# salesforce/warp-drive

Measured on AMD Instinct MI355X. Metric: env steps/sec, TagContinuous 5 taggers x 100 runners, higher is better.
Workload: dtype f32; 1 GPU; BASELINE configs[2]: TagContinuous 5 taggers x 100 runners, partial obs K=10 (F=71), num_envs=2000 per GPU; tick = sample_actions (2 heads) + step + reset of finished replicas (one fused launch); num_envs_per_gpu=2000, num_agents=105, launch_mode=plan, kernels_per_tick=1, ticks_per_launch=1, parallelism=env-replica sharding x1

## Files before the change

### experiments/phase_profile.py

```python
#!/usr/bin/env python3
import os
import subprocess
import sys

ROOT = os.path.dirname(os.path.dirname(os.path.abspath(__file__)))
sys.path.insert(0, ROOT)
PROF_DIR = os.environ.get("WD_PROF_DIR", os.path.join(ROOT, "build", "variants", "prof"))
if len(sys.argv) > 1 and sys.argv[1] == "build":
    from warp_drive_amd import build as wb

    if os.environ.get("WD_PROF_SRC"):
        wb.KDIR = os.environ["WD_PROF_SRC"]
        wb.KERNEL_FLAGS = [f"-I{wb.KDIR}" if f.startswith("-I") else f for f in wb.KERNEL_FLAGS]

    os.makedirs(PROF_DIR, exist_ok=True)
    for out, (unit, flags) in wb.UNITS.items():
        if out.startswith("wd_kernels_tc_k10"):
            subprocess.run([wb._hipcc(), *wb.KERNEL_FLAGS, *flags, "-DWD_TC_PROBES=1", os.path.join(wb.KDIR, unit), "-o",
                            os.path.join(PROF_DIR, out)], check=True)
            print("built", os.path.join(PROF_DIR, out))
    sys.exit(0)
E = int(sys.argv[1]) if len(sys.argv) > 1 else 2000
T_STAMP = int(sys.argv[2]) if len(sys.argv) > 2 else 300
N_RUNNERS = int(sys.argv[3]) if len(sys.argv) > 3 else 100
N_TICKS = int(sys.argv[4]) if len(sys.argv) > 4 else 32
name = "prof"
os.environ["WD_HSACO_DIR"] = PROF_DIR
os.environ.setdefault("HIP_FORCE_DEV_KERNARG", "1")
import time

import numpy as np
import torch

import bench
from warp_drive_amd.env_wrapper import EnvWrapper
from warp_drive_amd.envs.tag_continuous import TagContinuous
from warp_drive_amd.managers import hip_driver as drv
from warp_drive_amd.managers.function_manager import HIPSampler
from warp_drive_amd.rollout import RolloutEngine
from warp_drive_amd.training.data_loader import create_and_push_data_placeholders

w = EnvWrapper(env_obj=TagContinuous(**dict(bench.BENCH_CFG, num_runners=N_RUNNERS)), num_envs=E, env_backend="hip")
WPB = (w.n_agents + 63) // 64
w.reset_all_envs()
sampler = HIPSampler(w.cuda_function_manager)
sampler.init_random(seed=1)
create_and_push_data_placeholders(env_wrapper=w, action_sampler=sampler, training_batch_size_per_env=None,
                                  push_data_batch_placeholders=False)
engine = RolloutEngine(w, sampler, fused=True)
SLOTS = 24
n_waves = WPB * E
buf = drv.mem_alloc(n_waves * SLOTS * 8)
drv.memset(buf, 0, n_waves * SLOTS * 8)
sym, nbytes = w.cuda_function_manager._module_of(engine.step_kernel_name).get_global("tc_prof_g")
drv.memcpy_htod(sym, np.array([int(buf)], dtype=np.uint64))
engine.run(300)
torch.cuda.synchronize()
t0 = time.perf_counter()
engine.run(1000)
torch.cuda.synchronize()
print(f"=== {name}: wall per tick {(time.perf_counter() - t0) / 1000 * 1e6:.2f} us (stamped build)")
looped = engine.rollout_kernel_name is not None
stamp_trip = N_TICKS // 2 if looped else 0
engine.run((T_STAMP - stamp_trip - 1300) % 500)
torch.cuda.synchronize()
if looped:
    mod = w.cuda_function_manager._module_of(engine.rollout_kernel_name)
    drv.memcpy_htod(mod.get_global("tc_prof_g")[0], np.array([int(buf)], dtype=np.uint64))
    drv.memcpy_htod(mod.get_global("tc_prof_tick_g")[0], np.array([stamp_trip], dtype=np.int32))
    print(f"multi-tick entry {engine.rollout_kernel_name}: a launch of {N_TICKS} ticks, trip {stamp_trip} stamped "
          "(the wavefront counters add up over the whole launch)")
live = w.cuda_data_manager.pull_data_from_device("still_in_the_game").sum(axis=1).mean()
print(f"stamped launch = tick {T_STAMP} of an episode, {live:.1f} agents in the game")
drv.memset(buf, 0, n_waves * SLOTS * 8)
torch.cuda.synchronize()
engine.run(N_TICKS if looped else 1)
torch.cuda.synchronize()
raw = np.zeros(n_waves * SLOTS, dtype=np.uint64)
drv.memcpy_dtoh(raw, buf)
drv.synchronize()
st = raw.reshape(-1, SLOTS).astype(np.int64)
ran = st[:, 15] > 0
searched = st[:, 9] > 0
print(f"wavefronts: {ran.sum()}; ran the search: {searched.sum()}; with a lane in the two-pass fallback / whole-wavefront resolution: "
      f"{(st[:, 20] > 0).sum()}; with a lane whose close pair was settled by one exact compare: "
      f"{(st[:, 23] > 0).sum()}; with a lane in the full ranking: {(st[:, 22] > 0).sum()}")
pre = searched & (st[:, 19] > 0)
if pre.any():
    tr = st[pre, 18]
    print(f"prefiltered wavefronts: {pre.sum()}; radius check failed: {(st[pre, 19] == 2).sum()}; chain trips (pass 2) mean {tr.mean():.1f} "
          f"p50 {np.percentile(tr, 50):.0f} p99 {np.percentile(tr, 99):.0f} max {tr.max()}")
for k in range(1, 16):
    st[:, k] = np.where(st[:, k] > 0, st[:, k], st[:, k - 1])
names = ["start", "loads issued+tables", "sampled", "barrier1", "moved", "barrier2", "tags", "search: radius", "search: prefiltered chain",
         "search: full chain", "search: keys resolved", "search: ids, remember", "id rows + barrier + nearest ids flushed",
         "obs gathered+flushed", "barrier3", "rewards/end"]
if pre.any():
    sp = st[pre]
    print(f"--- all {pre.sum()} prefiltered wavefronts: mean / p10 / p50 / p90 / max shader cycles")
    for k in (7, 8, 9, 10, 11):
        d = sp[:, k] - sp[:, k - 1]
        print(f"  {names[k]:<40} {d.mean():9.0f} {np.percentile(d, 10):9.0f} {np.percentile(d, 50):9.0f} {np.percentile(d, 90):9.0f} {d.max():9.0f}")
    d = sp[:, 11] - sp[:, 6]
    print(f"  {'search, all of it':<40} {d.mean():9.0f} {np.percentile(d, 10):9.0f} {np.percentile(d, 50):9.0f} {np.percentile(d, 90):9.0f} {d.max():9.0f}")
    blk = np.nonzero(pre)[0] // WPB
    slow = np.array([d[blk == b].max() for b in np.unique(blk)])
    print(f"  slowest searcher of each block: mean {slow.mean():.0f} p50 {np.percentile(slow, 50):.0f} p90 {np.percentile(slow, 90):.0f}")
for wv, label in ((0, "wave 0 of each block"), (WPB - 1, "the last wave of each block")):
    s = st[wv::WPB]
    ok = (s[:, 6] > 0) & (s[:, 15] > 0)
    s = s[ok]
    print(f"--- {label}: {ok.sum()} waves; mean / p10 / p90 shader cycles per phase")
    for k in range(1, 16):
        d = s[:, k] - s[:, k - 1]
        print(f"  {names[k]:<40} {d.mean():9.0f} {np.percentile(d, 10):9.0f} {np.percentile(d, 90):9.0f}")
    tot = s[:, 15] - s[:, 0]
    real = (s[:, 17] - s[:, 16]) * 10.0
    print(f"  total {tot.mean():.0f} cycles = {real.mean() / 1000:.2f} us -> {tot.mean() / real.mean():.3f} GHz")
s = st[(st[:, 16] > 0) & (st[:, 17] > 0)]
t0 = s[:, 16].min()
start, end = (s[:, 16] - t0) / 100.0, (s[:, 17] - t0) / 100.0
pc = lambda a: " ".join(f"{np.percentile(a, q):6.2f}" for q in (0, 10, 50, 90, 99, 100))
print("percentiles 0/10/50/90/99/100 (us): wave start", pc(start), "| wave end", pc(end), "| lifetime", pc(end - start))
s0 = st[0::WPB]
s0 = s0[(s0[:, 6] > 0) & (s0[:, 15] > 0)]
ghz = ((s0[:, 15] - s0[:, 0]) / ((s0[:, 17] - s0[:, 16]) * 10.0)).mean()
base = (s0[:, 16] - t0) / 100.0
print("phase boundary, us since first wave start (p10 / p50 / p90), wave 0:")
for k in range(0, 16):
    tk = base + (s0[:, k] - s0[:, 0]) / (ghz * 1000.0)
    print(f"  {names[k]:<40} {np.percentile(tk, 10):7.2f} {np.percentile(tk, 50):7.2f} {np.percentile(tk, 90):7.2f}")

hw = st[:, 21]
okw = st[:, 15] > 0
simd_key = ((hw >> 32) & 15) * (1 << 20) + ((hw >> 13) & 7) * (1 << 16) + ((hw >> 12) & 1) * (1 << 12) + ((hw >> 8) & 15) * 16 + ((hw >> 4) & 3)
role = np.arange(len(st)) % WPB
endt = (st[:, 17] - t0) / 100.0
import collections
per = collections.defaultdict(list)
# ... 31 lines not shown
```

### warp_drive_amd/csrc/kernels/tag_continuous.hip

```cpp
#include "wd_common.h"

#include "tc_types.h"
#include "tc_fetch.h"
#include "tc_sample.h"
#include "tc_move.h"
#include "tc_tags.h"
#include "tc_reset.h"
#include "tc_knn.h"
#include "tc_rows.h"
#include "tc_fast.h"
#include "tc_generic.h"

#define WD_TC_PARAMS                                                                              \
  float *loc_x_arr, float *loc_y_arr, float *speed_arr, float *direction_arr,                     \
      float *acceleration_arr, const int *agent_types_arr, float *edge_hit_reward_penalty,        \
      float kEdgeHitPenalty, float kGridLength, const float *acceleration_actions_arr,            \
      const float *turn_actions_arr, float kMaxSpeed, int kNumOtherAgentsObserved,                \
      const float *skill_levels_arr, int kRunnerExitsGameAfterTagged, int *still_in_the_game_arr, \
      int kUseFullObservation, float *obs_arr, const int *action_indices_arr,                     \
      float *neighbor_distances_arr, int *neighbor_ids_sorted_by_distance_arr,                    \
      int *nearest_neighbor_ids, float *rewards_arr, const float *step_rewards_arr,               \
      int *num_runners_arr, float kDistanceMarginForReward, float kTagRewardForTagger,            \
      float kTagPenaltyForRunner, float kEndOfGameRewardForRunner, int *done_arr,                 \
      int *env_timestep_arr, int kNumAgents, int kEpisodeLength, int kNumEnvs,                    \
      int kNumAccelerationActions, int kNumTurnActions, int *obs_rows_cleared_arr,                 \
      unsigned *knn_prev_arr, int kEnvBegin

#define WD_TC_PACK()                                                                              \
  TcArgs a;                                                                                       \
  a.loc_x = loc_x_arr; a.loc_y = loc_y_arr; a.speed = speed_arr; a.direction = direction_arr;     \
  a.acceleration = acceleration_arr; a.agent_types = agent_types_arr;                             \
  a.edge_pen_arr = edge_hit_reward_penalty; a.edge_hit_penalty = kEdgeHitPenalty;                 \
  a.grid_length = kGridLength; a.acc_actions = acceleration_actions_arr;                          \
  a.turn_actions = turn_actions_arr; a.max_speed = kMaxSpeed; a.K = kNumOtherAgentsObserved;      \
  a.skill_levels = skill_levels_arr; a.runner_exits = kRunnerExitsGameAfterTagged;                \
  a.sig_arr = still_in_the_game_arr; a.use_full_obs = kUseFullObservation; a.obs = obs_arr;       \
  a.actions = action_indices_arr; a.nearest_ids = nearest_neighbor_ids; a.rewards = rewards_arr;  \
  a.step_rewards = step_rewards_arr; a.num_runners = num_runners_arr;                             \
  a.margin = kDistanceMarginForReward; a.tag_reward = kTagRewardForTagger;                        \
  a.tag_penalty = kTagPenaltyForRunner; a.end_reward = kEndOfGameRewardForRunner;                 \
  a.done = done_arr; a.timestep = env_timestep_arr; a.N = kNumAgents; a.T = kEpisodeLength;       \
  a.E = kNumEnvs; a.env_begin = kEnvBegin; a.obs_rows_cleared = obs_rows_cleared_arr;              \
  a.knn_prev = knn_prev_arr;                                                                      \
  (void)neighbor_distances_arr; (void)neighbor_ids_sorted_by_distance_arr;

#define WD_TC_FUSE_PARAMS                                                                      \
  , uint32_t *rng_state, const float *probs_acc, const float *probs_turn, const void *reset_table, \
      int n_reset_arrays, int stream_tag
#define WD_TC_FUSE_PACK()                                                                      \
  TcFuse fz;                                                                                   \
  fz.rng_state = rng_state; fz.probs_acc = probs_acc; fz.probs_turn = probs_turn;              \
  fz.actions_out = const_cast<int *>(action_indices_arr);                                      \
  fz.reset_table = (const wd_reset_entry *)reset_table; fz.n_reset_arrays = n_reset_arrays;      \
  fz.stream_tag = stream_tag;

extern "C" {

#define WD_TC_CAT_(a, b) a##b
#define WD_TC_CAT(a, b) WD_TC_CAT_(a, b)
#define WD_TC_SMEM() extern __shared__ __attribute__((aligned(16))) unsigned char tc_smem[]

#if !defined(WD_TC_KM)

__global__ void HipTagContinuousStep(WD_TC_PARAMS) {
  WD_TC_SMEM();
  WD_TC_PACK();
  tc_generic_impl<false>(a, TcFuse{}, tc_smem, kNumAccelerationActions, kNumTurnActions);
}

__global__ void HipTagContinuousTick(WD_TC_PARAMS WD_TC_FUSE_PARAMS) {
  WD_TC_SMEM();
  WD_TC_PACK();
  WD_TC_FUSE_PACK();
  tc_generic_impl<true>(a, fz, tc_smem, kNumAccelerationActions, kNumTurnActions);
}

#elif defined(WD_TC_SHAPE_N)

#define WD_TC_SHAPE_NAME(stem) WD_TC_CAT(WD_TC_CAT(WD_TC_CAT(WD_TC_CAT(WD_TC_CAT(stem, WD_TC_KM), _N), WD_TC_SHAPE_N), A), WD_TC_SHAPE_A)
static_assert(WD_TC_SHAPE_N <= 128, "the shape-specialised entries use the 7-bit-id search of replicas up to 128 agents");
#if defined(WD_TC_ROLLOUT)
static_assert(WD_TC_SHAPE_N > 64 && WD_TC_SHAPE_THREADS == 128, "one replica per 128-thread block");
__global__ void __launch_bounds__(512, 4) WD_TC_SHAPE_NAME(HipTagContinuousRollout_K)(WD_TC_PARAMS WD_TC_FUSE_PARAMS,
                                                                                      int kNumTicks) {
  WD_TC_SMEM();
  WD_TC_PACK();
  WD_TC_FUSE_PACK();
  a.N = WD_TC_SHAPE_N; a.K = WD_TC_KM;
  tc_fast_rollout<WD_TC_KM, true, 7, WD_TC_SHAPE_N, WD_TC_SHAPE_A, WD_TC_SHAPE_THREADS>(a, fz, tc_smem, WD_TC_SHAPE_A,
                                                                                        WD_TC_SHAPE_A, kNumTicks);
}
#else
__global__ void __launch_bounds__(512, 4) WD_TC_SHAPE_NAME(HipTagContinuousStep_K)(WD_TC_PARAMS) {
  WD_TC_SMEM();
  WD_TC_PACK();
  a.N = WD_TC_SHAPE_N; a.K = WD_TC_KM;
  tc_fast_impl<WD_TC_KM, false, true, 7>(a, TcFuse{}, tc_smem, WD_TC_SHAPE_A, WD_TC_SHAPE_A);
}
__global__ void __launch_bounds__(512, 4) WD_TC_SHAPE_NAME(HipTagContinuousTick_K)(WD_TC_PARAMS WD_TC_FUSE_PARAMS) {
  WD_TC_SMEM();
  WD_TC_PACK();
  WD_TC_FUSE_PACK();
  a.N = WD_TC_SHAPE_N; a.K = WD_TC_KM;
  tc_fast_impl<WD_TC_KM, true, true, 7>(a, fz, tc_smem, WD_TC_SHAPE_A, WD_TC_SHAPE_A);
}
__global__ void __launch_bounds__(512, 4) WD_TC_SHAPE_NAME(HipTagContinuousTickA_K)(WD_TC_PARAMS WD_TC_FUSE_PARAMS) {
  WD_TC_SMEM();
  WD_TC_PACK();
  WD_TC_FUSE_PACK();
  a.N = WD_TC_SHAPE_N; a.K = WD_TC_KM;
  tc_fast_impl<WD_TC_KM, true, true, 7, false>(a, fz, tc_smem, WD_TC_SHAPE_A, WD_TC_SHAPE_A);
}
#endif

#else

#define WD_TC_NAME(stem, suffix) WD_TC_CAT(WD_TC_CAT(stem, WD_TC_KM), suffix)
#define WD_TC_FAST_ENTRIES(suffix, THREADS, WAVES, IDB, SPLIT_EXACT)                                            \
  __global__ void __launch_bounds__(THREADS, WAVES) WD_TC_NAME(HipTagContinuousStep_K, suffix)(WD_TC_PARAMS) {   \
    WD_TC_SMEM();                                                                                                \
    WD_TC_PACK();                                                                                                \
    if (SPLIT_EXACT && a.K == WD_TC_KM)                                                                          \
      tc_fast_impl<WD_TC_KM, false, SPLIT_EXACT, IDB>(a, TcFuse{}, tc_smem, kNumAccelerationActions, kNumTurnActions); \
    else                                                                                                         \
      tc_fast_impl<WD_TC_KM, false, false, IDB>(a, TcFuse{}, tc_smem, kNumAccelerationActions, kNumTurnActions); \
  }                                                                                                              \
  __global__ void __launch_bounds__(THREADS, WAVES) WD_TC_NAME(HipTagContinuousTick_K, suffix)(WD_TC_PARAMS WD_TC_FUSE_PARAMS) { \
    WD_TC_SMEM();                                                                                                \
    WD_TC_PACK();                                                                                                \
// ... 22 lines not shown
```

### warp_drive_amd/csrc/kernels/tc_config.h

```cpp
#pragma once
#include "wd_common.h"

#if defined(WD_TC_SHAPE_THREADS)
#define WD_TC_BLOCKDIM WD_TC_SHAPE_THREADS
#else
#define WD_TC_BLOCKDIM ((int)blockDim.x)
#endif

#ifdef WD_TC_PROBES
extern "C" { __device__ unsigned long long *tc_prof_g = nullptr; }
extern "C" { __device__ int tc_prof_tick_g = 0; }
#define WD_TC_PROBE_TICK(loop, tick) const bool tc_prof_on = !(loop) || (tick) == tc_prof_tick_g
#define WD_TC_SLOT(k) ((blockIdx.x * (blockDim.x >> 6) + (threadIdx.x >> 6)) * 24 + (k))
#define WD_TC_PROBE(k) do { if ((threadIdx.x & 63) == 0 && tc_prof_g && tc_prof_on) tc_prof_g[WD_TC_SLOT(k)] = __builtin_readcyclecounter(); } while (0)
#define WD_TC_PROBE_RT(k) do { if ((threadIdx.x & 63) == 0 && tc_prof_g && tc_prof_on) tc_prof_g[WD_TC_SLOT(k)] = __builtin_amdgcn_s_memrealtime(); } while (0)
#define WD_TC_PROBE_VAL(k, v) do { if (tc_prof_g) { const unsigned long long m_ = __ballot(1);                          \
    if ((threadIdx.x & 63) == (unsigned)(__ffsll((long long)m_) - 1)) tc_prof_g[WD_TC_SLOT(k)] += (unsigned long long)(v); } } while (0)
#define WD_TC_PROBE_HW(k) do { if ((threadIdx.x & 63) == 0 && tc_prof_g && tc_prof_on) { unsigned hw_, xcc_;                        \
    asm volatile("s_getreg_b32 %0, hwreg(HW_REG_HW_ID)" : "=s"(hw_));                                                    \
    asm volatile("s_getreg_b32 %0, hwreg(HW_REG_XCC_ID)" : "=s"(xcc_));                                                  \
    tc_prof_g[WD_TC_SLOT(k)] = (unsigned long long)hw_ | ((unsigned long long)(xcc_ & 15u) << 32); } } while (0)
#else
#define WD_TC_PROBE_TICK(loop, tick)
#define WD_TC_PROBE_HW(k)
#define WD_TC_PROBE(k)
#define WD_TC_PROBE_RT(k)
#define WD_TC_PROBE_VAL(k, v)
#endif
```

### warp_drive_amd/csrc/kernels/tc_fast.h

```cpp
#pragma once
#include "wd_common.h"
#include "tc_fetch.h"
#include "tc_sample.h"
#include "tc_move.h"
#include "tc_tags.h"
#include "tc_reset.h"
#include "tc_knn.h"
#include "tc_rows.h"

namespace {

template <int KMAX, bool FUSED, bool EXACTK, int IDB, bool SAMPLE = FUSED, bool LOOP = false, int SN = 0, int SA = 0,
          int ST = 0>
__device__ __forceinline__ int tc_fast_impl(const TcArgs &a, const TcFuse &fz, unsigned char *smem, int n_acc,
                                            int n_turn, int tick = 0, int n_taggers_in = 0, TcCarry *cy = nullptr) {
  WD_TC_PROBE_TICK(LOOP, tick);
  const int N = a.N, K = EXACTK ? KMAX : a.K;
  const int F = 7 * K + 1;
  int tid_ = threadIdx.x;
  if constexpr (LOOP) asm volatile("" : "+v"(tid_));
  const int tid = tid_, T_ = WD_TC_BLOCKDIM;
  const int epb = max(1, T_ / N);
  const int n_waves = (T_ + 63) >> 6, wave = __builtin_amdgcn_readfirstlane(tid >> 6), lane = tid & 63;
  const size_t slab_acc_bytes = tc_align16((size_t)4 * epb * N * n_acc);
  const bool compact = (epb == 1);
  const size_t slab_turn_bytes = tc_align16((size_t)4 * epb * N * n_turn);
  const bool one_slab = tc_one_slab(N);
  const TcFastLds l = tc_carve_fast(smem, epb, N, K, n_waves,
                                    !SAMPLE ? 0 : one_slab ? max(slab_acc_bytes, slab_turn_bytes) : slab_acc_bytes + slab_turn_bytes,
                                    compact);
  const TcTables &tb = l.tb;
  float *const slab_acc = (float *)smem, *const slab_turn = (float *)(smem + (one_slab ? 0 : slab_acc_bytes));
  float *const stage = l.stage + (size_t)wave * l.stage_dwords;
  const int el = tid / N, ag = tid - el * N;
  const float invK = 1.0f / (float)K, invN = 1.0f / (float)N;
  const int NP = ((N + 3) & ~3) + 8;

  int group = blockIdx.x;
#ifndef WD_TC_BLOCK_ORDER_PLAIN
  if constexpr (IDB == 7) {
    const int bx = blockIdx.x & 7, bq = gridDim.x >> 3, br = gridDim.x & 7;
    group = bx * bq + min(bx, br) + (int)(blockIdx.x >> 3);
  }
#endif
  const int env0 = a.env_begin + group * epb;
  __builtin_amdgcn_s_setprio(3);
  WD_TC_PROBE_RT(16); WD_TC_PROBE(0); WD_TC_PROBE_HW(21);
  TcIn in;
  bool reloaded = false;
  if constexpr (LOOP) {
    in = cy->in;
    reloaded = cy->reload != 0;
    if (reloaded) {
      tc_load_state(in, a, fz, env0, epb, N, n_acc, n_turn, tid, tick == 0);
      cy->in.type = in.type; cy->in.skill = in.skill; cy->in.step_reward = in.step_reward;
    }
  } else {
    tc_issue_loads<FUSED, SAMPLE>(in, a, fz, env0, epb, N, n_acc, n_turn, tid, slab_acc, slab_turn, true);
  }
  const bool tab_in_lds = (n_acc <= WD_TC_TAB) && (n_turn <= WD_TC_TAB);
  int n_taggers_ = n_taggers_in;
  if constexpr (LOOP) {
    if (tick == 0) n_taggers_ = tc_build_tables(tb, a, N, n_acc, n_turn, tab_in_lds, in);
  } else {
    n_taggers_ = tc_build_tables(tb, a, N, n_acc, n_turn, tab_in_lds, in);
  }
  const int n_taggers = n_taggers_;
  if (env0 >= a.E) return n_taggers;
// ... 15 lines not shown
  if constexpr (!LOOP) {
    if (compact && lane == 0) tb.live_cnt[wave] = __popcll(live_mask);
  }
  if constexpr ((IDB != 7) && (KMAX <= 12)) {
    if (compact && tid < 64) tb.cell_cnt[tid] = 0;
  }
  if constexpr (LOOP) {
    static_assert(!LOOP || IDB == 7, "tc_sample_heads_carried samples from two slabs: replicas of at most 128 agents");
    sampled = tc_sample_heads_carried(fz, in.epoch, cy->k0, cy->k1, active, gi, li, slab_acc, slab_turn, n_acc, n_turn);
    if (compact && lane == 0) tb.live_cnt[wave] = __popcll(live_mask);
  } else if (FUSED) {
    if (active && ag == 0) a.done[env] = 0;
    if (SAMPLE) sampled = tc_sample_heads(a, fz, in, active, gi, li, slab_acc, slab_turn, n_acc, n_turn, env0, epb);
  }
  WD_TC_PROBE(2);
  __syncthreads();
  WD_TC_PROBE(3);
  int my_c = ag, n_live = N;
  if (compact) {
    int before = 0;
    n_live = 0;
    for (int w2 = 0; w2 < n_waves; ++w2) {
      const int c = tb.live_cnt[w2];
      before += (w2 < wave) ? c : 0;
      n_live += c;
    }
    my_c = before + __popcll(live_mask & ((1ull << lane) - 1ull));
  }
  constexpr bool PRE = (IDB != 7) && (KMAX <= 12);
  constexpr bool TIE_TABLE = (IDB != 7);
  bool pre_on = false;
  int cells_C = 0;
  float cell_len = 0.0f, cell_inv = 0.0f;
  int my_cell = 0, my_cell_slot = 0;
  uint4 hint_a = make_uint4(~0u, ~0u, ~0u, ~0u), hint_b = hint_a;
  if constexpr (PRE) {
    pre_on = compact && (a.knn_prev != nullptr) && (n_live >= WD_TC_PRE_MIN_LIVE) && (l.stage_dwords >= WD_TC_LIST_DWORDS);
    if (pre_on && active && in.sg != 0) {
      const uint4 *const h = (const uint4 *)(a.knn_prev + (size_t)(env * N + ag) * 8);
      hint_a = h[0];
      hint_b = h[1];
    }
    if (pre_on) {
      cells_C = tc_cell_grid(n_live, K);
      cell_len = a.grid_length / (float)max(cells_C, 1);
      cell_inv = (float)cells_C / a.grid_length;
    }
  }

  float edge_pen = 0.0f, my_x = 0.0f, my_y = 0.0f;
  const int sg = in.sg;
  const bool is_runner = active && (in.type == 0) && (sg != 0);
  if (active) {
    const TcMoved m = tc_move(a, tb, in, sampled, gi, tab_in_lds, LOOP ? cy : nullptr);
    edge_pen = m.edge_pen; my_x = m.x; my_y = m.y;
    if constexpr (LOOP) {
      cy->in.x = m.x; cy->in.y = m.y;
      cy->in.cleared = (sg == 0) ? 1 : 0;
    }
    l.xy[el * NP + ag] = make_float2(sg ? m.x : (PRE && pre_on ? __builtin_nanf("") : WD_BIG), m.y);
    if (compact) {
      if (sg) {
        bool by_cell = false;
        if constexpr (PRE) {
          if (cells_C != 0) {
            const int2 c = tc_cell_xy(m.x, m.y, cell_inv, cells_C);
            my_cell = tc_cell_place(c, cells_C);
            my_cell_slot = atomicAdd(&tb.cell_cnt[my_cell], 1);
            by_cell = true;
          }
        }
        if (!by_cell) {
          l.xyc[my_c] = make_float2(m.x, m.y);
          l.cid[1 + my_c] = (short)ag;
          if (PRE && pre_on) {
            uint4 *const slot = (uint4 *)(l.stage + (size_t)(my_c >> 6) * l.stage_dwords) + 2 * (my_c & 63);
            slot[0] = hint_a;
            slot[1] = hint_b;
          }
        }
      }
      if (ag == 0) {
        l.cid[0] = -1;
        if (PRE && pre_on) {
          l.xyc[n_live] = make_float2(WD_BIG, WD_BIG);
          l.xy[N] = make_float2(__builtin_nanf(""), 0.0f);
        }
      }
    }
    tc_feat_store(l.feat, li, m.ft);
    l.sig[li] = (sg ? 1 : 0) | (in.cleared ? 2 : 0);
    if ((in.cleared != 0) != (sg == 0)) a.obs_rows_cleared[gi] = sg ? 0 : 1;
    l.tagcnt[li] = 0;
    if (ag == 0) {
      const int t = in.tstep + 1;
      a.timestep[env] = t;
      tb.tstep[el] = t;
      tb.tfrac[el] = (float)((double)t / (double)a.T);
      if constexpr (LOOP) {
        cy->in.tstep = t;
        if (reloaded) tb.nrun[el] = in.nrun;
      } else {
        tb.nrun[el] = in.nrun;
      }
    }
  }
  WD_TC_PROBE(4);
  __syncthreads();
  WD_TC_PROBE(5);
  int cell_incl = 0;
  if constexpr (PRE) {
    if (cells_C != 0) {
      const int cnt = tb.cell_cnt[lane];
      cell_incl = cnt;
#pragma unroll
      for (int d = 1; d < 64; d <<= 1) {
        const int up = __shfl_up(cell_incl, d, 64);
        cell_incl += (lane >= d) ? up : 0;
      }
      my_c = __builtin_amdgcn_ds_bpermute(my_cell << 2, cell_incl - cnt) + my_cell_slot;
      if (active && sg != 0) {
        l.xyc[my_c] = make_float2(my_x, my_y);
        l.cid[1 + my_c] = (short)ag;
        uint4 *const slot = (uint4 *)(l.stage + (size_t)(my_c >> 6) * l.stage_dwords) + 2 * (my_c & 63);
        slot[0] = hint_a;
        slot[1] = hint_b;
      }
    }
  }

  bool tagged = false;
  if (is_runner)
    tagged = tc_find_tag(a, tb, l.xy + el * NP, l.tagcnt + el * N, &tb.nrun[el], n_taggers, my_x, my_y);
  if constexpr (PRE) {
    if (cells_C != 0) __syncthreads();
  }

  WD_TC_PROBE(6);
  int nid[KMAX + 1], rank[KMAX + 1];
#pragma unroll
  for (int k = 0; k <= KMAX; ++k) { nid[k] = -1; rank[k] = k; }
  bool in_order = true;
  __builtin_amdgcn_s_setprio(2);
  const bool searcher = compact ? (tid < n_live) : (active && sg != 0);
  const float2 *const sxy = compact ? l.xyc : l.xy + el * NP;
  const int n_cand = compact ? n_live : N;
  int row_agent = ag;
  constexpr int L = KMAX + ((EXACTK && IDB == 7) ? 2 : 3);
  const bool split = compact && (n_waves == 2) && (n_live <= 64) && (n_live >= 16) &&
                     (l.stage_dwords >= 64 * L);
  const int j_half = split ? (((n_live + 7) >> 3) << 2) : n_cand;
  const bool helper = split && (wave == 1);
  unsigned S[L];
  bool prefiltered = false;
  unsigned extra = 0xffffffffu;
  if constexpr (PRE) {
    if (pre_on) {
      unsigned Tb = 0u;
      float sx = 0.0f, sy = 0.0f;
      int2 scell = make_int2(0, 0);
      if (searcher) {
        const uint4 *const slot = (const uint4 *)stage + 2 * lane;
        const uint4 pa = slot[0], pb = slot[1];
        sx = sxy[ag].x; sy = sxy[ag].y;
        Tb = tc_knn_bound16<KMAX>(l.xy, N, sx, sy, pa, pb, K);
        if (cells_C != 0) {
          scell = tc_cell_xy(sx, sy, cell_inv, cells_C);
          Tb = min(Tb, tc_cell_cover2(sx, sy, scell, cell_len, cells_C));
        }
      }
      WD_TC_PROBE(7);
      if (__ballot(searcher) != 0ull && __ballot(searcher && Tb == 0x7f800000u) == 0ull) {
        const float Tf = searcher ? __uint_as_float(Tb) : -1.0f;
#pragma unroll
        for (int k = 0; k < L; ++k) S[k] = 0xffffffffu;
        const int C = cells_C;
        int r = 0, r_end = -1, run0 = 0, run1 = n_cand, x_lo = 0, y_lo = 0, x_hi = 0, y_hi = 0;
        if (C != 0) {
          const int last = min(63, __builtin_amdgcn_readfirstlane(n_live) - 1 - 64 * wave);
          x_lo = __builtin_amdgcn_readfirstlane(scell.x); y_lo = __builtin_amdgcn_readfirstlane(scell.y);
          x_hi = __builtin_amdgcn_readlane(scell.x, last); y_hi = __builtin_amdgcn_readlane(scell.y, last);
          r = max(0, y_lo - 1);
          r_end = min(C - 1, y_hi + 1);
          run1 = 0;
        }
        const TcPreList pl = tc_pre_list(stage, lane);
// ... 263 lines not shown
        o[6 * K] = __uint_as_float((0u - (ts & 1u)) & 0x3f800000u);
      }
      if (lane < rc) {
        const int m = wrow0 + r0 + lane;
        const int e_m = (int)(((float)m + 0.5f) * invN);
        stage[mis + lane * F + 7 * K] = (l.sig[m] & 1) ? tb.tfrac[e_m] : 0.0f;
      }
      asm volatile("" ::: "memory");
      __builtin_amdgcn_wave_barrier();
      tc_flush_run(stage, dst, rc * F, lane);
      asm volatile("" ::: "memory");
      __builtin_amdgcn_wave_barrier();
    }
  }
  WD_TC_PROBE(13);
  __syncthreads();
  WD_TC_PROBE(14);

  if (active) tc_finish_agent(a, tb, el, ag, gi, env, sg, is_runner, tagged, l.tagcnt[li], edge_pen, in.step_reward, FUSED);
  if (FUSED) {
    __syncthreads();
    bool any = false;
    for (int e = 0; e < min(epb, a.E - env0); ++e) any = any || (tb.doneflag[e] != 0);
    if constexpr (LOOP) {
      if (active) {
        cy->in.sg = (tagged && a.runner_exits) ? 0 : sg;
        cy->in.epoch = in.epoch + 1u;
      }
      cy->reload = __builtin_amdgcn_readfirstlane(any ? 1 : 0);
    }
    if (any) {
      asm volatile("s_waitcnt vmcnt(0)" ::: "memory");
      __syncthreads();
      tc_reset_finished(a, fz, tb, env0, epb);
      if constexpr (LOOP) {
        asm volatile("s_waitcnt vmcnt(0)" ::: "memory");
        __syncthreads();
      }
    }
  }
  WD_TC_PROBE(15); WD_TC_PROBE_RT(17);
  return n_taggers;
}

template <int KMAX, bool EXACTK, int IDB, int SN, int SA, int ST>
__device__ __forceinline__ void tc_fast_rollout(const TcArgs &a, const TcFuse &fz, unsigned char *smem, int n_acc,
                                                int n_turn, int ticks) {
  int n_taggers = 0;
  TcCarry cy;
  cy.in = TcIn{};
  cy.reload = 1;
  cy.k0 = __builtin_amdgcn_readfirstlane(fz.rng_state[0]);
  cy.k1 = __builtin_amdgcn_readfirstlane(fz.rng_state[1]);
  for (int tick = 0; tick < ticks; ++tick) {
    n_taggers = tc_fast_impl<KMAX, true, EXACTK, IDB, true, true, SN, SA, ST>(a, fz, smem, n_acc, n_turn, tick, n_taggers, &cy);
    asm volatile("s_waitcnt vmcnt(0)" ::: "memory");
    __syncthreads();
  }
}

}
```

### warp_drive_amd/csrc/kernels/tc_move.h

```cpp
#pragma once
#include "wd_common.h"
#include "tc_types.h"

namespace {

__device__ __forceinline__ float tc_remainder_two_pi(float a, float b) {
  const float aa = fabsf(a);
  if (__builtin_expect(__ballot(!(aa < 2.0f * b)) != 0ull, 0)) return wd_np_remainderf(a, b);
  float m = aa - ((aa >= b) ? b : 0.0f);
  m = (a < 0.0f && m != 0.0f) ? b - m : m;
  return m;
}

struct TcMoved {
  float x, y, edge_pen;
  TcFeat ft;
};
__device__ __forceinline__ TcMoved tc_move(const TcArgs &a, const TcTables &tb, const TcIn &in, int2 act, int gi,
                                           bool tab_in_lds, TcCarry *cy = nullptr) {
  const float two_pi = 6.2831854820251465f;
  const float L = a.grid_length;
  const double diag = (double)L * 1.4142135623730951;
  const float sp_div = a.max_speed + 1.0e-10f;
  const float s = (float)in.sg;
  float d_acc = tb.acc_tab[min(act.x, WD_TC_TAB - 1)], d_turn = tb.turn_tab[min(act.y, WD_TC_TAB - 1)];
  asm volatile("" : "+v"(d_acc), "+v"(d_turn));
  if (!tab_in_lds) {
    d_acc = a.acc_actions[act.x];
    d_turn = a.turn_actions[act.y];
  }
  const float dir = tc_remainder_two_pi(in.dir + d_turn, two_pi) * s;
  float acc = in.acc + d_acc;
  const float vmax = a.max_speed * in.skill;
  float v = in.speed + acc;
  v = fminf(fmaxf(v, 0.0f), vmax) * s;
  acc = acc * (v > 0.0f ? 1.0f : 0.0f) * (v < vmax ? 1.0f : 0.0f);
  float sn, cs;
  wd_np_sincosf(dir, sn, cs);
  float px = in.x + v * cs;
  float py = in.y + v * sn;
  const bool crossed = !((px >= 0.0f) && (px <= L) && (py >= 0.0f) && (py <= L));
  px = fminf(fmaxf(px, 0.0f), L);
  py = fminf(fmaxf(py, 0.0f), L);
  TcMoved m;
  m.edge_pen = a.edge_hit_penalty * (crossed ? 1.0f : 0.0f);
  a.loc_x[gi] = px;
  a.loc_y[gi] = py;
  a.speed[gi] = v;
  a.direction[gi] = dir;
  a.acceleration[gi] = acc;
  a.edge_pen_arr[gi] = m.edge_pen;
  m.x = px;
  m.y = py;
  if (cy != nullptr) { cy->in.dir = dir; cy->in.acc = acc; cy->in.speed = v; }
  m.ft.nx = (double)px / diag;
  m.ft.ny = (double)py / diag;
  m.ft.nsp = v / sp_div;
  m.ft.nac = acc / sp_div;
  m.ft.ndir = dir / two_pi;
  m.ft.type_sig = ((in.type & 1) ? 0x3f800000 : 0) | (in.sg ? 1 : 0);
  return m;
}

__device__ __forceinline__ void tc_obs_values(float (&vals)[7], const TcFeat &nb, const TcFeat &me, bool rel,
                                              bool valid) {
  unsigned mr = rel ? 0xffffffffu : 0u, mv = valid ? 0xffffffffu : 0u;
  asm volatile("" : "+v"(mr), "+v"(mv));
  vals[0] = __uint_as_float(__float_as_uint((float)(nb.nx - me.nx)) & mr);
  vals[1] = __uint_as_float(__float_as_uint((float)(nb.ny - me.ny)) & mr);
  vals[2] = __uint_as_float(__float_as_uint(nb.nsp - me.nsp) & mr);
  vals[3] = __uint_as_float(__float_as_uint(nb.nac - me.nac) & mr);
  vals[4] = __uint_as_float(__float_as_uint(nb.ndir - me.ndir) & mr);
  const unsigned one = 0x3f800000u, ts = (unsigned)nb.type_sig;
  vals[5] = __uint_as_float(ts & one & mv);
  vals[6] = __uint_as_float((0u - (ts & 1u)) & one & mv);
}

}
```

### warp_drive_amd/csrc/kernels/tc_tags.h

```cpp
#pragma once
#include "wd_common.h"
#include "tc_types.h"

namespace {

__device__ __forceinline__ bool tc_find_tag(const TcArgs &a, const TcTables &tb, const float2 *cxy, int *tagcnt_env,
                                            int *nrun_env, int n_taggers, float my_x, float my_y) {
  float best = __builtin_inff();
  int bt = -1;
  constexpr int U = 5;
  for (int t0 = 0; t0 < n_taggers; t0 += U) {
    int j[U];
    float2 pt[U];
#pragma unroll
    for (int u = 0; u < U; ++u) j[u] = tb.tagger_ids[min(t0 + u, n_taggers - 1)];
#pragma unroll
    for (int u = 0; u < U; ++u) pt[u] = cxy[j[u]];
#pragma unroll
    for (int u = 0; u < U; ++u) {
      const float dx = my_x - pt[u].x, dy = my_y - pt[u].y;
      const float d = sqrtf(dx * dx + dy * dy);
      if (t0 + u < n_taggers && d < best) { best = d; bt = j[u]; }
    }
  }
  if (bt >= 0 && best < a.margin) {
    atomicAdd(&tagcnt_env[bt], 1);
    if (a.runner_exits) atomicSub(nrun_env, 1);
    return true;
  }
  return false;
}

__device__ __forceinline__ void tc_finish_agent(const TcArgs &a, const TcTables &tb, int el, int ag, int gi, int env,
                                                int sg, bool is_runner, bool tagged, int tagcnt, float edge_pen,
                                                float step_reward, bool fused) {
  float rew = 0.0f;
  if (sg) { rew += edge_pen; rew += step_reward; }
  if (tagged) rew += a.tag_penalty;
  for (int k = 0; k < tagcnt; ++k) rew += a.tag_reward;
  const bool still_runner = is_runner && !(tagged && a.runner_exits);
  if (tb.tstep[el] == a.T && still_runner) rew += a.end_reward;
  a.rewards[gi] = rew;
  if (tagged && a.runner_exits) a.sig_arr[gi] = 0;
  if (ag == 0) {
    const int nr = tb.nrun[el];
    a.num_runners[env] = nr;
    const bool fin = (tb.tstep[el] >= a.T || nr == 0);
    if (fin) a.done[env] = 1;
    if (fused) tb.doneflag[el] = fin ? 1 : 0;
  }
}

}
```

### warp_drive_amd/envs/tag_continuous.py

```python
import copy
import os

import numpy as np

from warp_drive_amd.utils import spaces
from warp_drive_amd.utils.constants import Constants
from warp_drive_amd.utils.data_feed import DataFeed
from warp_drive_amd.utils.gpu_environment_context import CUDAEnvironmentContext

_OBSERVATIONS = Constants.OBSERVATIONS
_ACTIONS = Constants.ACTIONS
_REWARDS = Constants.REWARDS
_LOC_X, _LOC_Y, _SP, _DIR, _ACC, _SIG = "loc_x", "loc_y", "speed", "direction", "acceleration", "still_in_the_game"

_K_SPECIALISATIONS = (2, 4, 6, 8, 10, 12, 16, 24, 32)

f32 = np.float32


class TagContinuous(CUDAEnvironmentContext):
    name = "TagContinuous"
    RESET_IS_DETERMINISTIC = True

    def __init__(self, num_taggers=1, num_runners=10, grid_length=10.0, episode_length=100,
# ... 320 lines not shown
    def _range_args(self, env_range):
        args = list(self.cuda_step_function_feed(self._STEP_ARGS))
        epb, block, grid = self._geometry()
        if env_range is None:
            return args + [np.int32(0)], epb, block, grid
        begin, end = int(env_range[0]), int(env_range[1])
        n_envs_pos = self._STEP_ARGS.index(("n_envs", "meta"))
        args[n_envs_pos] = np.int32(end)
        grid = (max(1, min(grid[0], (end - begin + epb - 1) // epb)), 1)
        return args + [np.int32(begin)], epb, block, grid

    def step_launch(self, env_range=None):
        args, epb, block, grid = self._range_args(env_range)
        return self.cuda_step, args, block, grid, self.lds_bytes(epb, threads=block[0])

    LDS_PER_WORKGROUP = 160 * 1024

    def can_fuse_tick(self):
        epb, block, _ = self._geometry()
        return self.lds_bytes(epb, fused=True, threads=block[0]) <= self.LDS_PER_WORKGROUP

    def has_presampled_tick(self):
        name = self.cuda_step.name.replace("Step", "TickA")
        return self._fast_path() and self.cuda_function_manager.has_function(name)

    TICK_ENV_RANGES = True

    def tick_launch(self, sampler, probabilities, resetter, env_range=None):
        from warp_drive_amd.managers.function_manager import _stream_tag

        fm, dm = self.cuda_function_manager, self.cuda_data_manager
        presampled = probabilities is None
        name = self.cuda_step.name.replace("Step", "TickA" if presampled else "Tick")
        fm.initialize_functions([name])
        fn = fm.get_function(name)
        _, reset_args, _, _ = resetter.fused_launch(dm, 0, 0)
        table, n_arrays = reset_args[0], reset_args[1]
        args, epb, block, grid = self._range_args(env_range)
        if presampled:
            null = np.uint64(0)
            args = args + [null, null, null, table, n_arrays, _stream_tag("tick")]
            return fn, args, block, grid, self.lds_bytes(epb, fused=False, threads=block[0])
        assert len(probabilities) == 2
        args = args + [sampler.rng_state, probabilities[0], probabilities[1], table, n_arrays, _stream_tag("tick")]
        return fn, args, block, grid, self.lds_bytes(epb, fused=True, threads=block[0])

    def rollout_launch(self, sampler, probabilities, resetter):
        if not self._fast_path() or "Step" not in self.cuda_step.name:
            return None
        fm = self.cuda_function_manager
        name = self.cuda_step.name.replace("Step", "Rollout")
        if not fm.has_function(name):
            return None
        _, args, block, grid, shared = self.tick_launch(sampler, probabilities, resetter)
        fm.initialize_functions([name])
        return fm.get_function(name), args + [np.int32(1)], block, grid, shared

    def step(self, actions=None):
        self.timestep += 1
        if self.env_backend != "cpu":
            fn, args, block, grid, shared = self.step_launch()
            fn(*args, block=block, grid=grid, shared=shared)
            return None
        assert isinstance(actions, dict) and len(actions) == self.num_agents
        acc_ids = [actions[a][0] for a in range(self.num_agents)]
        turn_ids = [actions[a][1] for a in range(self.num_agents)]
        assert all(0 <= i <= self.num_acceleration_levels for i in acc_ids)
        assert all(0 <= i <= self.num_turn_levels for i in turn_ids)
        self.update_state(self.acceleration_actions[acc_ids], self.turn_actions[turn_ids])
        obs = self.generate_observation()
        rew = self.compute_reward()
        done = {"__all__": (self.timestep >= self.episode_length) or (self.num_runners == 0)}
        return obs, rew, done, {}
```

Before: 119.5 million env_steps/s.

## Replace loop-invariant divisions with reciprocal-FMA and skip far tagger groups in rollout

In the looped rollout path, the per-agent divisions by max speed, grid diagonal, 2π and episode length are replaced with a multiply-by-reciprocal plus one FMA correction step. The reciprocals are precomputed once per launch, and a wavefront-wide fallback to true division runs for out-of-class inputs. A one-time GPU kernel checks every float input exhaustively for bit-exactness and disables the rollout path if any mismatch is found. The tag search also compares squared distances against a margin bound and skips a whole unrolled group of taggers when no lane in the wavefront is within range, avoiding the sqrt work. The price is a costly one-off verification sweep, extra code paths and ballots.

```diff
diff --git a/experiments/phase_profile.py b/experiments/phase_profile.py
--- a/experiments/phase_profile.py
+++ b/experiments/phase_profile.py
@@ -16,7 +16,8 @@
     os.makedirs(PROF_DIR, exist_ok=True)
     for out, (unit, flags) in wb.UNITS.items():
         if out.startswith("wd_kernels_tc_k10"):
-            subprocess.run([wb._hipcc(), *wb.KERNEL_FLAGS, *flags, "-DWD_TC_PROBES=1", os.path.join(wb.KDIR, unit), "-o",
+            subprocess.run([wb._hipcc(), *wb.KERNEL_FLAGS, *flags, f"-DWD_TC_PROBES={int(os.environ.get('WD_PROF_LEVEL', '1'))}",
+                            os.path.join(wb.KDIR, unit), "-o",
                             os.path.join(PROF_DIR, out)], check=True)
             print("built", os.path.join(PROF_DIR, out))
     sys.exit(0)
@@ -85,6 +86,10 @@
 print(f"wavefronts: {ran.sum()}; ran the search: {searched.sum()}; with a lane in the two-pass fallback / whole-wavefront resolution: "
       f"{(st[:, 20] > 0).sum()}; with a lane whose close pair was settled by one exact compare: "
       f"{(st[:, 23] > 0).sum()}; with a lane in the full ranking: {(st[:, 22] > 0).sum()}")
+if looped and st[:, 18].any():
+    for wv in range(WPB):
+        sk = st[wv::WPB][ran[wv::WPB], 18]
+        print(f"tag roots skipped, wave {wv}: {sk.sum()} of {len(sk) * N_TICKS} wavefront-trips ({sk.sum() / max(1, len(sk) * N_TICKS):.4f})")
 pre = searched & (st[:, 19] > 0)
 if pre.any():
     tr = st[pre, 18]
diff --git a/warp_drive_amd/csrc/kernels/tag_continuous.hip b/warp_drive_amd/csrc/kernels/tag_continuous.hip
--- a/warp_drive_amd/csrc/kernels/tag_continuous.hip
+++ b/warp_drive_amd/csrc/kernels/tag_continuous.hip
@@ -75,6 +75,44 @@
   tc_generic_impl<true>(a, fz, tc_smem, kNumAccelerationActions, kNumTurnActions);
 }
 
+__global__ void HipTagContinuousVerifyInvariantDivide(float kMaxSpeed, float kGridLength, int kEpisodeLength, int *res) {
+  const TcLoopConsts lc = tc_loop_consts(kMaxSpeed, kGridLength, kEpisodeLength, 0.0f);
+  const float sp_div = tc_sp_div(kMaxSpeed);
+  const double diag = tc_diag(kGridLength), Td = (double)kEpisodeLength;
+  const uint32_t gtid = blockIdx.x * blockDim.x + threadIdx.x, gsize = gridDim.x * blockDim.x;
+  if (gtid == 0) {
+    const bool sane = sp_div > 0.0f && sp_div < __builtin_inff() && diag > 0.0 && diag < (double)__builtin_inff() &&
+                      kEpisodeLength > 0;
+    if (!sane) res[0] = 0;
+    res[5] = 2;
+  }
+  int bad_sp = 0, bad_pi = 0, bad_diag = 0, bad_T = 0, in_class = 0;
+  for (uint64_t i = gtid; i < (1ull << 32); i += gsize) {
+    const float x = __uint_as_float((uint32_t)i);
+    if (tc_div_const_in_class(x, 0.0f, 0.0f)) {
+      ++in_class;
+      const float w0 = x / sp_div, g0 = tc_div_const(x, sp_div, lc.r_sp);
+      const float w1 = x / WD_TC_TWO_PI, g1 = tc_div_const(x, WD_TC_TWO_PI, WD_TC_R_TWO_PI);
+      bad_sp += (__float_as_uint(w0) != __float_as_uint(g0)) && !(w0 != w0 && g0 != g0);
+      bad_pi += (__float_as_uint(w1) != __float_as_uint(g1)) && !(w1 != w1 && g1 != g1);
+    }
+    if ((__float_as_uint(x) & 0x7fffffffu) != 0x7f800000u) {
+      const double xd = (double)x, w = xd / diag, g = tc_div_const(xd, diag, lc.r_diag);
+      bad_diag += (__double_as_longlong(w) != __double_as_longlong(g)) && !(w != w && g != g);
+    }
+  }
+  for (int t = 1 + (int)gtid; t <= kEpisodeLength && t > 0; t += (int)min(gsize, 0x40000000u)) {
+    const float w = (float)((double)t / Td), g = (float)tc_div_const((double)t, Td, lc.r_T);
+    bad_T += __float_as_uint(w) != __float_as_uint(g);
+  }
+  if (bad_sp) atomicAdd(&res[1], bad_sp);
+  if (bad_pi) atomicAdd(&res[2], bad_pi);
+  if (bad_diag) atomicAdd(&res[3], bad_diag);
+  if (bad_T) atomicAdd(&res[4], bad_T);
+  if (bad_sp | bad_pi | bad_diag | bad_T) res[0] = 0;
+  if (in_class) atomicAdd((unsigned long long *)(res + 6), (unsigned long long)in_class);
+}
+
 #elif defined(WD_TC_SHAPE_N)
 
 #define WD_TC_SHAPE_NAME(stem) WD_TC_CAT(WD_TC_CAT(WD_TC_CAT(WD_TC_CAT(WD_TC_CAT(stem, WD_TC_KM), _N), WD_TC_SHAPE_N), A), WD_TC_SHAPE_A)
diff --git a/warp_drive_amd/csrc/kernels/tc_config.h b/warp_drive_amd/csrc/kernels/tc_config.h
--- a/warp_drive_amd/csrc/kernels/tc_config.h
+++ b/warp_drive_amd/csrc/kernels/tc_config.h
@@ -20,7 +20,13 @@
     asm volatile("s_getreg_b32 %0, hwreg(HW_REG_HW_ID)" : "=s"(hw_));                                                    \
     asm volatile("s_getreg_b32 %0, hwreg(HW_REG_XCC_ID)" : "=s"(xcc_));                                                  \
     tc_prof_g[WD_TC_SLOT(k)] = (unsigned long long)hw_ | ((unsigned long long)(xcc_ & 15u) << 32); } } while (0)
+#if WD_TC_PROBES >= 2
+#define WD_TC_PROBE_TAG_SKIP() WD_TC_PROBE_VAL(18, 1)
 #else
+#define WD_TC_PROBE_TAG_SKIP()
+#endif
+#else
+#define WD_TC_PROBE_TAG_SKIP()
 #define WD_TC_PROBE_TICK(loop, tick)
 #define WD_TC_PROBE_HW(k)
 #define WD_TC_PROBE(k)
diff --git a/warp_drive_amd/csrc/kernels/tc_divide.h b/warp_drive_amd/csrc/kernels/tc_divide.h
--- /dev/null
+++ b/warp_drive_amd/csrc/kernels/tc_divide.h
@@ -0,0 +1,43 @@
+#pragma once
+#include "wd_common.h"
+
+namespace {
+
+__device__ __forceinline__ float tc_div_const(float x, float y, float r) {
+  const float q0 = x * r;
+  const float e = __builtin_fmaf(q0, y, -x);
+  return __builtin_fmaf(-e, r, q0);
+}
+__device__ __forceinline__ double tc_div_const(double x, double y, double r) {
+  const double q0 = x * r;
+  const double e = __builtin_fma(q0, y, -x);
+  return __builtin_fma(-e, r, q0);
+}
+
+__device__ __forceinline__ bool tc_div_const_in_class(float a, float b, float c) {
+  const int lo = min(min(__builtin_amdgcn_frexp_expf(a), __builtin_amdgcn_frexp_expf(b)), __builtin_amdgcn_frexp_expf(c));
+  const float sum = fabsf(a) + fabsf(b) + fabsf(c);
+  return (sum < 0x1.0p64f) && (lo >= -64);
+}
+
+struct TcLoopConsts {
+  float r_sp;
+  double r_diag;
+  double r_T;
+  float Bc;
+};
+#define WD_TC_TWO_PI 6.2831854820251465f
+#define WD_TC_R_TWO_PI (1.0f / WD_TC_TWO_PI)
+__device__ __forceinline__ float tc_sp_div(float max_speed) { return max_speed + 1.0e-10f; }
+__device__ __forceinline__ double tc_diag(float grid_length) { return (double)grid_length * 1.4142135623730951; }
+__device__ __forceinline__ TcLoopConsts tc_loop_consts(float max_speed, float grid_length, int T, float margin) {
+  TcLoopConsts c;
+  c.r_sp = 1.0f / tc_sp_div(max_speed);
+  c.r_diag = 1.0 / tc_diag(grid_length);
+  c.r_T = 1.0 / (double)T;
+  const float b = (margin * margin) * 0x1.00001p0f;
+  c.Bc = (b > 0.0f) ? __uint_as_float(__float_as_uint(b) + 1u) : b;
+  return c;
+}
+
+}
diff --git a/warp_drive_amd/csrc/kernels/tc_fast.h b/warp_drive_amd/csrc/kernels/tc_fast.h
--- a/warp_drive_amd/csrc/kernels/tc_fast.h
+++ b/warp_drive_amd/csrc/kernels/tc_fast.h
@@ -13,7 +13,8 @@
 template <int KMAX, bool FUSED, bool EXACTK, int IDB, bool SAMPLE = FUSED, bool LOOP = false, int SN = 0, int SA = 0,
           int ST = 0>
 __device__ __forceinline__ int tc_fast_impl(const TcArgs &a, const TcFuse &fz, unsigned char *smem, int n_acc,
-                                            int n_turn, int tick = 0, int n_taggers_in = 0, TcCarry *cy = nullptr) {
+                                            int n_turn, int tick = 0, int n_taggers_in = 0, TcCarry *cy = nullptr,
+                                            const TcLoopConsts *lc = nullptr) {
   WD_TC_PROBE_TICK(LOOP, tick);
   const int N = a.N, K = EXACTK ? KMAX : a.K;
   const int F = 7 * K + 1;
@@ -135,7 +136,7 @@
   const int sg = in.sg;
   const bool is_runner = active && (in.type == 0) && (sg != 0);
   if (active) {
-    const TcMoved m = tc_move(a, tb, in, sampled, gi, tab_in_lds, LOOP ? cy : nullptr);
+    const TcMoved m = tc_move<LOOP>(a, tb, in, sampled, gi, tab_in_lds, LOOP ? cy : nullptr, LOOP ? lc : nullptr);
     edge_pen = m.edge_pen; my_x = m.x; my_y = m.y;
     if constexpr (LOOP) {
       cy->in.x = m.x; cy->in.y = m.y;
@@ -179,7 +180,8 @@
       const int t = in.tstep + 1;
       a.timestep[env] = t;
       tb.tstep[el] = t;
-      tb.tfrac[el] = (float)((double)t / (double)a.T);
+      if constexpr (LOOP) tb.tfrac[el] = (float)tc_div_const((double)t, (double)a.T, lc->r_T);
+      else tb.tfrac[el] = (float)((double)t / (double)a.T);
       if constexpr (LOOP) {
         cy->in.tstep = t;
         if (reloaded) tb.nrun[el] = in.nrun;
@@ -213,8 +215,13 @@
   }
 
   bool tagged = false;
-  if (is_runner)
-    tagged = tc_find_tag(a, tb, l.xy + el * NP, l.tagcnt + el * N, &tb.nrun[el], n_taggers, my_x, my_y);
+  if constexpr (LOOP) {
+    if (is_runner)
+      tagged = tc_find_tag<true>(a, tb, l.xy + el * NP, l.tagcnt + el * N, &tb.nrun[el], n_taggers, my_x, my_y, lc->Bc);
+  } else {
+    if (is_runner)
+      tagged = tc_find_tag(a, tb, l.xy + el * NP, l.tagcnt + el * N, &tb.nrun[el], n_taggers, my_x, my_y);
+  }
   if constexpr (PRE) {
     if (cells_C != 0) __syncthreads();
   }
@@ -584,8 +591,10 @@
   cy.reload = 1;
   cy.k0 = __builtin_amdgcn_readfirstlane(fz.rng_state[0]);
   cy.k1 = __builtin_amdgcn_readfirstlane(fz.rng_state[1]);
+  const TcLoopConsts lc = tc_loop_consts(a.max_speed, a.grid_length, a.T, a.margin);
   for (int tick = 0; tick < ticks; ++tick) {
-    n_taggers = tc_fast_impl<KMAX, true, EXACTK, IDB, true, true, SN, SA, ST>(a, fz, smem, n_acc, n_turn, tick, n_taggers, &cy);
+    n_taggers = tc_fast_impl<KMAX, true, EXACTK, IDB, true, true, SN, SA, ST>(a, fz, smem, n_acc, n_turn, tick, n_taggers, &cy,
+                                                                              &lc);
     asm volatile("s_waitcnt vmcnt(0)" ::: "memory");
     __syncthreads();
   }
diff --git a/warp_drive_amd/csrc/kernels/tc_move.h b/warp_drive_amd/csrc/kernels/tc_move.h
--- a/warp_drive_amd/csrc/kernels/tc_move.h
+++ b/warp_drive_amd/csrc/kernels/tc_move.h
@@ -1,6 +1,7 @@
 #pragma once
 #include "wd_common.h"
 #include "tc_types.h"
+#include "tc_divide.h"
 
 namespace {
 
@@ -16,8 +17,9 @@
   float x, y, edge_pen;
   TcFeat ft;
 };
+template <bool CDIV = false>
 __device__ __forceinline__ TcMoved tc_move(const TcArgs &a, const TcTables &tb, const TcIn &in, int2 act, int gi,
-                                           bool tab_in_lds, TcCarry *cy = nullptr) {
+                                           bool tab_in_lds, TcCarry *cy = nullptr, const TcLoopConsts *lc = nullptr) {
   const float two_pi = 6.2831854820251465f;
   const float L = a.grid_length;
   const double diag = (double)L * 1.4142135623730951;
@@ -53,11 +55,24 @@
   m.x = px;
   m.y = py;
   if (cy != nullptr) { cy->in.dir = dir; cy->in.acc = acc; cy->in.speed = v; }
-  m.ft.nx = (double)px / diag;
-  m.ft.ny = (double)py / diag;
-  m.ft.nsp = v / sp_div;
-  m.ft.nac = acc / sp_div;
-  m.ft.ndir = dir / two_pi;
+  if constexpr (CDIV) {
+    m.ft.nx = tc_div_const((double)px, diag, lc->r_diag);
+    m.ft.ny = tc_div_const((double)py, diag, lc->r_diag);
+    m.ft.nsp = tc_div_const(v, sp_div, lc->r_sp);
+    m.ft.nac = tc_div_const(acc, sp_div, lc->r_sp);
+    m.ft.ndir = tc_div_const(dir, two_pi, WD_TC_R_TWO_PI);
+    if (__builtin_expect(__ballot(!tc_div_const_in_class(v, acc, dir)) != 0ull, 0)) {
+      m.ft.nsp = v / sp_div;
+      m.ft.nac = acc / sp_div;
+      m.ft.ndir = dir / two_pi;
+    }
+  } else {
+    m.ft.nx = (double)px / diag;
+    m.ft.ny = (double)py / diag;
+    m.ft.nsp = v / sp_div;
+    m.ft.nac = acc / sp_div;
+    m.ft.ndir = dir / two_pi;
+  }
   m.ft.type_sig = ((in.type & 1) ? 0x3f800000 : 0) | (in.sg ? 1 : 0);
   return m;
 }
diff --git a/warp_drive_amd/csrc/kernels/tc_tags.h b/warp_drive_amd/csrc/kernels/tc_tags.h
--- a/warp_drive_amd/csrc/kernels/tc_tags.h
+++ b/warp_drive_amd/csrc/kernels/tc_tags.h
@@ -4,8 +4,9 @@
 
 namespace {
 
+template <bool SKIP = false>
 __device__ __forceinline__ bool tc_find_tag(const TcArgs &a, const TcTables &tb, const float2 *cxy, int *tagcnt_env,
-                                            int *nrun_env, int n_taggers, float my_x, float my_y) {
+                                            int *nrun_env, int n_taggers, float my_x, float my_y, float Bc = 0.0f) {
   float best = __builtin_inff();
   int bt = -1;
   constexpr int U = 5;
@@ -16,11 +17,33 @@
     for (int u = 0; u < U; ++u) j[u] = tb.tagger_ids[min(t0 + u, n_taggers - 1)];
 #pragma unroll
     for (int u = 0; u < U; ++u) pt[u] = cxy[j[u]];
+    if constexpr (!SKIP) {
 #pragma unroll
-    for (int u = 0; u < U; ++u) {
-      const float dx = my_x - pt[u].x, dy = my_y - pt[u].y;
-      const float d = sqrtf(dx * dx + dy * dy);
-      if (t0 + u < n_taggers && d < best) { best = d; bt = j[u]; }
+      for (int u = 0; u < U; ++u) {
+        const float dx = my_x - pt[u].x, dy = my_y - pt[u].y;
+        const float d = sqrtf(dx * dx + dy * dy);
+        if (t0 + u < n_taggers && d < best) { best = d; bt = j[u]; }
+      }
+    } else {
+      float d2[U];
+#pragma unroll
+      for (int u = 0; u < U; ++u) {
+        const float dx = my_x - pt[u].x, dy = my_y - pt[u].y;
+        d2[u] = dx * dx + dy * dy;
+      }
+      unsigned lo = 0x7f800000u, hi = 0u;
+#pragma unroll
+      for (int u = 0; u < U; ++u) { lo = min(lo, __float_as_uint(d2[u])); hi = max(hi, __float_as_uint(d2[u])); }
+      const float m2 = __uint_as_float(hi > 0x7f800000u ? hi : lo);
+      if (__ballot(!(m2 > Bc)) == 0ull) {
+        WD_TC_PROBE_TAG_SKIP();
+        continue;
+      }
+#pragma unroll
+      for (int u = 0; u < U; ++u) {
+        const float d = sqrtf(d2[u]);
+        if (t0 + u < n_taggers && d < best) { best = d; bt = j[u]; }
+      }
     }
   }
   if (bt >= 0 && best < a.margin) {
diff --git a/warp_drive_amd/envs/tag_continuous.py b/warp_drive_amd/envs/tag_continuous.py
--- a/warp_drive_amd/envs/tag_continuous.py
+++ b/warp_drive_amd/envs/tag_continuous.py
@@ -396,9 +396,32 @@
         name = self.cuda_step.name.replace("Step", "Rollout")
         if not fm.has_function(name):
             return None
+        if not self.invariant_divide_ok():
+            return None
         _, args, block, grid, shared = self.tick_launch(sampler, probabilities, resetter)
         fm.initialize_functions([name])
         return fm.get_function(name), args + [np.int32(1)], block, grid, shared
+
+    _INVARIANT_DIVIDE_VERDICTS = {}
+
+    def invariant_divide_verdict(self):
+        key = (float(self.max_speed), float(self.grid_length), int(self.episode_length))
+        cache = TagContinuous._INVARIANT_DIVIDE_VERDICTS
+        if key not in cache:
+            import torch
+
+            fm = self.cuda_function_manager
+            fm.initialize_functions(["HipTagContinuousVerifyInvariantDivide"])
+            res = torch.zeros(8, dtype=torch.int32, device=torch.device("cuda", torch.cuda.current_device()))
+            res[0] = 1
+            fm.get_function("HipTagContinuousVerifyInvariantDivide")(
+                np.float32(self.max_speed), np.float32(self.grid_length), np.int32(self.episode_length), res,
+                block=(256, 1, 1), grid=(8192, 1), shared=0)
+            cache[key] = [int(v) for v in res.cpu().numpy()]
+        return cache[key]
+
+    def invariant_divide_ok(self):
+        return self.invariant_divide_verdict()[0] == 1
 
     def step(self, actions=None):
         self.timestep += 1
```

Measured after the change: 124.1 million env_steps/s (median of 6 runs). +3.9%, better.
